# MarwanNour/SEAL-FYP-Logistic-Regression

Measured on AMD Instinct MI355X. Metric: CKKS ciphertext rotate+plain-mult ops/sec at N=16384; HBM GB/s vs roofline, higher is better.
Workload: dtype u64; 1 GPU; C3: N=16384, coeff_modulus bits [60, 40, 40, 40, 40, 60], level L=5 (k=6); per step and per GPU 4608 independent rotate_vector(step=1, direct Galois key)+multiply_plain, uniform random residues drawn on the device, inputs resident in HBM; batch_per_gpu=4608, parallelism=1 x independent ciphertext batches (no data-path collective), algorithmic_bytes_per_op=11141120

## Files before the change

seal_fyp_logistic_regression_amd/csrc/hefx_capi.cpp:

```cpp
#include "../../include/hefx.h"

#include <chrono>
#include <cmath>
#include <cstdio>
#include <cstring>
#include <map>
#include <mutex>
#include <tuple>
#include <string>
#include <unordered_map>
#include <unordered_set>
#include <algorithm>
#include <functional>
#include <vector>

#include <dlfcn.h>
#include <link.h>

#include "hefx_internal.h"

using namespace hefx;
typedef unsigned __int128 u128;

static thread_local std::string g_err;
// ... 981 lines not shown
        if (e == hipSuccess) rc = ntt_common(c, false, (uint64_t *)(rows + per * i0), cnt, c->k, 0, (void *)s);
    }
    if (e == hipSuccess && rc == HEFX_OK) e = hipStreamSynchronize(s);
    if (e != hipSuccess || rc != HEFX_OK) {
        (void)hipFree(rows);
        return rc != HEFX_OK ? rc : hipfail(e, "flip-mask tables");
    }
    std::lock_guard<std::mutex> lk(c->mu);
    c->flipw_slabs.push_back(rows);
    c->flipw_bytes += per * miss.size() * sizeof(u64);
    for (size_t i = 0; i < miss.size(); ++i) c->flipw.emplace(miss[i], rows + per * i);
    resolve();
    return HEFX_OK;
}

static size_t ks_words_per_item(const hefx_context *c, int L)
{
    return (size_t)c->n * ((size_t)L + 2 * (size_t)(L + 1) + 2);
}
static size_t ks_x_words(const hefx_context *c, int L, int items) { return (size_t)c->n * items * L * (L + 1); }

static int ks_small_shape(int n, int L)
{
    static const int quarter_force = getenv("HEFX_QUARTER") ? atoi(getenv("HEFX_QUARTER")) : -1;
    static const int qmask_force = getenv("HEFX_QMASK") ? atoi(getenv("HEFX_QMASK")) : -1;
    static const int pair_force = getenv("HEFX_PAIR") ? atoi(getenv("HEFX_PAIR")) : -1;
    if (qmask_force >= 0) return qmask_force & (KS_Q_ALL | KS_Q_PAIR);
    if (pair_force > 0 || (pair_force < 0 && quarter_force < 0 && n * L * L * 4 <= 256)) return KS_Q_PAIR;
    if (quarter_force >= 0) return quarter_force ? KS_Q_ALL : 0;
    return (n * L * 4 <= 256 ? KS_Q_INTT : 0) | (n * L * L * 4 <= 256 ? KS_Q_NTT : 0) | (n * 2 * 4 <= 256 ? KS_Q_MDI : 0) |
           (n * 2 * L * 4 <= 320 ? KS_Q_FIN : 0);
// ... 6 lines not shown
{
    CTXCHK(c);
    static const bool ksdbg = getenv("HEFX_DEBUG") && atoi(getenv("HEFX_DEBUG")) >= 2;
    const auto ks_t0 = std::chrono::steady_clock::now();
    auto ks_us = [&] { return std::chrono::duration<double, std::micro>(std::chrono::steady_clock::now() - ks_t0).count(); };
    double t_valid = 0, t_tables = 0;
    if (int rc = check_ks_level(c, L)) return rc;
    if (n < 1 || !ct_in || !ct_out) return fail(HEFX_ERR_INVALID, "bad key-switch batch arguments");
    if (!relin && (!elts || !keys)) return fail(HEFX_ERR_INVALID, "missing Galois elements / keys");
    if (relin && !single_key) return fail(HEFX_ERR_INVALID, "missing relinearization key");
    if ((acc_in != nullptr) != (acc_out != nullptr) || (acc_out && (relin || pts || hoist)))
        return fail(HEFX_ERR_INVALID, "accumulate: rotations only, input and output sums together, no fused plaintext");
    const size_t per = ks_words_per_item(c, L);
    int chunk = c->chunk;
    if (chunk <= 0) {
        chunk = (int)(((size_t)1 << 30) / (per * sizeof(u64)));
        const int cap = c->logn <= 13 ? 2 * KS_AUTO_CHUNK : KS_AUTO_CHUNK;
        chunk = chunk > cap ? cap : (chunk < 16 ? 16 : chunk & ~7);
    }
    const int nchunks = (n + chunk - 1) / chunk;
    const bool two = nchunks > 1 && c->use_streams && !c->profiling;
    if (hoist) {
        if (relin) return fail(HEFX_ERR_INVALID, "hoisting applies to rotations only");
        for (int i = 0; i < n; ++i)
            if (ct_in[i] != ct_in[0] || ct_out[i] == ct_in[0])
                return fail(HEFX_ERR_INVALID, "hoisted batch: one shared source, never overwritten");
    }
    std::vector<const uint32_t *> perms(relin ? 0 : (size_t)n);
    bool any_alias = false;
    for (int i = 0; i < n; ++i) {
        if (!ct_in[i] || !ct_out[i]) return fail(HEFX_ERR_INVALID, "null ciphertext pointer in batch");
// ... 112 lines not shown
    }
    int ci = 0;
    ++c->stat_ks_calls;
    for (int base = 0; base < n && herr == hipSuccess; base += chunk, ++ci) {
        const int cnt = (n - base < chunk) ? n - base : chunk;
        const unsigned slot = c->ring_next++ % KS_RING;
        if (c->ring_busy[slot]) {
            KS_TRY(hipEventSynchronize(c->ring_ev[slot]));
            c->ring_busy[slot] = false;
        }
        KsItem *hb = c->h_items + (size_t)slot * KS_MAX_CHUNK, *db = c->d_items + (size_t)slot * KS_MAX_CHUNK;
        KsScratch S{};
        S.d = c->scratch + scratch_off + (two ? (size_t)(ci % ns) * half_words : 0);
        S.acc = S.d + (size_t)cnt * L * N;
        S.u = S.acc + (size_t)cnt * 2 * (L + 1) * N;
        S.x = S.u + (size_t)cnt * 2 * N;
        S.alias = S.x + ks_x_words(c, L, cnt);
        S.qmod = c->d_qmod;
        S.gate = c->d_gate + slot;
        S.gate_hits = c->d_gate + KS_RING;
        if (++c->gate_seq == 0) c->gate_seq = 1;
        S.gate_tag = c->gate_seq;
        S.gate_mode = 0;
        bool chunk_alias = false;
        int nsrc = 0;
        std::unordered_map<const void *, uint32_t> src_of;
        if (share && cnt > ks_small_max() && one_source && cnt + 1 <= KS_MAX_CHUNK) {
            src_of.emplace((const void *)ct_in[0], 0u);
            nsrc = 1;
        } else if (share && cnt > ks_small_max()) {
            for (int i = 0; i < cnt && src_of.size() * share_ratio <= (size_t)cnt; ++i)
// ... 189 lines not shown
        KsScratch S;
        KsItem *dbA, *dbB;
        hipStream_t s;
    };
    Lane lane[MAX_LANES];
    size_t off = 0;
    for (int l = 0; l < nl; ++l) {
        Lane &ln = lane[l];
        ln.lo = (int)((long long)n * l / nl);
        ln.cnt = (int)((long long)n * (l + 1) / nl) - ln.lo;
        ln.quarter = ks_small_shape(ln.cnt, L);
        ln.S = KsScratch{};
        ln.S.d = c->scratch + off;
        ln.S.acc = ln.S.d + (size_t)ln.cnt * L * N;
        ln.S.u = ln.S.acc + (size_t)ln.cnt * 2 * (L + 1) * N;
        ln.S.x = ln.S.u + (size_t)ln.cnt * 2 * N;
        ln.S.alias = ln.S.x + ks_x_words(c, L, ln.cnt);
        off += per * (size_t)ln.cnt + ks_x_words(c, L, ln.cnt);
        ln.dbA = c->chain_items + (size_t)l * 128;
        ln.dbB = ln.dbA + 64;
        ln.s = l == 0 ? user : c->streams[l - 1];
    }
    hipError_t herr = hipSuccess;
    if (nl > 1) {
        herr = hipEventRecord(c->ev_fork, user);
        for (int l = 1; l < nl && herr == hipSuccess; ++l) herr = hipStreamWaitEvent(lane[l].s, c->ev_fork, 0);
    }
    auto lane_level = [&](const Lane &ln, const uint64_t *const *in, uint64_t *const *out, KsItem *db) {
        return chain_level(c, L, ln.cnt, in + ln.lo, out + ln.lo, acc_out + ln.lo, acc_out + ln.lo, elts + ln.lo, keys + ln.lo,
                           perms.data() + ln.lo, ln.S, db, ln.quarter, ln.s);
    };
// ... 576 lines not shown
            for (int q = 1; q < LANES; ++q)
                if (load[q] < load[ln]) ln = q;
            root_lane[(size_t)r] = (uint8_t)ln;
            load[ln] += weight[(size_t)r];
        }
        std::vector<int> cnt((size_t)max_depth * LANES, 0);
        int widest = 0;
        for (size_t i = 0; i < nodes.size(); ++i) {
            lane_of[i] = root_lane[(size_t)root_of[i]];
            widest = std::max(widest, ++cnt[(size_t)nodes[i].depth * LANES + lane_of[i]]);
        }
        bool all_loaded = true;
        for (int q = 0; q < LANES; ++q) all_loaded = all_loaded && load[q] > 0;
        int chunk = c->chunk;
        if (chunk <= 0) {
            chunk = (int)(((size_t)1 << 30) / (ks_words_per_item(c, L) * sizeof(u64)));
            const int cap = c->logn <= 13 ? 2 * KS_AUTO_CHUNK : KS_AUTO_CHUNK;
            chunk = chunk > cap ? cap : (chunk < 16 ? 16 : chunk & ~7);
        }
        if (all_loaded && widest <= chunk) {
            lane1_off = ks_words_per_item(c, L) * (size_t)widest + ks_x_words(c, L, widest);
            if (int rc = ensure_scratch(c, (size_t)LANES * lane1_off)) return rc;
            nlanes = LANES;
            std::vector<uint32_t> all_elts(nodes.size());
            for (size_t i = 0; i < nodes.size(); ++i) all_elts[i] = nodes[i].elt;
            std::sort(all_elts.begin(), all_elts.end());
            all_elts.erase(std::unique(all_elts.begin(), all_elts.end()), all_elts.end());
            std::vector<const u64 *> unused;
            if (int rc = ensure_flipw(c, all_elts.data(), (int)all_elts.size(), (hipStream_t)stream, unused)) return rc;
            for (uint32_t e : all_elts) {
                const uint32_t *perm = nullptr;
// ... 354 lines not shown
        if (int rc = ks_run(c, L, 1, false, &src, &first[t], &key, nullptr, nullptr, &dst, stream)) return rc;
        src = dst;
    }
    if (int rc = hefx_add(c, L, 2, 1, ct, src, ct_new, stream)) return rc;
    if (int rc = hefx_multiply_plain(c, L, 2, 1, ct_new, diag_pts_keylevel[0], cbuf, stream)) return rc;
    if (nrot == 0) {
        HIPCHK(hipMemcpyAsync(out, cbuf, ctw * sizeof(u64), hipMemcpyDeviceToDevice, (hipStream_t)stream));
        return HEFX_OK;
    }
    const size_t per = ks_words_per_item(c, L) + ks_x_words(c, L, 1);
    if (int rc = ensure_scratch(c, per)) return rc;
    KsScratch S{};
    S.d = c->scratch;
    S.acc = S.d + (size_t)L * N;
    S.u = S.acc + (size_t)2 * (L + 1) * N;
    S.x = S.u + (size_t)2 * N;
    S.alias = nullptr;
    hipStream_t s = (hipStream_t)stream;
    HIPCHK(hipMemcpyAsync(d_items, items.data(), sizeof(KsItem) * items.size(), hipMemcpyHostToDevice, s));
    HIPCHK(hipStreamSynchronize(s));
    HIPCHK(launch_lt2_decompose(c->T, L, d_items, d_items + 1, nrot, S, (const u64 *)ct_new, partial_s, partial_c0,
                                (u64 *)cbuf, s));
    HIPCHK(launch_lt2_moddown(c->T, L, d_items + nterms, S, s));
    return HEFX_OK;
}

extern "C" int hefx_linear_transform_plain_hoisted2(hefx_context *c, int L, const uint64_t *ct, int d,
                                                    const uint64_t *const *diag_pts_keylevel, int nkeys,
                                                    const uint32_t *key_elts, const uint64_t *const *keys,
                                                    uint64_t *out, void *stream)
{
// ... 243 lines not shown
```

seal_fyp_logistic_regression_amd/csrc/hefx_keyswitch.hip:

```cpp
#include <cstdio>
#include <cstdlib>
#include "hefx_internal.h"
#include "hefx_ntt.cuh"
#include "hefx_ntt8.cuh"

template <int LOGN>
struct KsWaves {
    static constexpr int INV = LOGN <= 14 ? 2 : 4;
    static constexpr int FWD = LOGN <= 13 ? 2 : 4;
    static constexpr int NB_INV = (INV <= 2 && LOGN <= 13) ? 1 : 2, NB_FWD = (FWD <= 2 && LOGN < 13) ? 1 : 2;
    static constexpr bool PARITY_CUT = true;
};

namespace hefx {

typedef u64 u64x2_t __attribute__((ext_vector_type(2)));
__device__ __forceinline__ ulonglong2 nt_load16(const u64 *p)
{
    const u64x2_t v = __builtin_nontemporal_load(reinterpret_cast<const u64x2_t *>(p));
    return make_ulonglong2(v.x, v.y);
}
__device__ __forceinline__ void nt_store16(u64 *p, u64 a, u64 b)
{
    u64x2_t v;
    v.x = a, v.y = b;
    __builtin_nontemporal_store(v, reinterpret_cast<u64x2_t *>(p));
// ... 715 lines not shown
    const size_t w = (size_t)blockIdx.x * blockDim.x + threadIdx.x;
    u64 xl = 0, xh = 0, yl = 0, yh = 0;
    const int l0 = ch * LT2_CHUNK, l1 = l0 + LT2_CHUNK < nrot ? l0 + LT2_CHUNK : nrot;
    const u64 *__restrict__ row = c0 + (size_t)j * n;
    for (int l = l0; l < l1; ++l) {
        const KsItem it = items[l];
        const uint2 pi = gld_u32x2(it.perm + 2 * w);
        const ulonglong2 dg = gld16(it.pt + (size_t)j * n + 2 * w);
        mac128(xl, xh, gld8(row + pi.x), dg.x);
        mac128(yl, yh, gld8(row + pi.y), dg.y);
    }
    reinterpret_cast<ulonglong2 *>(partial + ((size_t)ch * L + j) * n)[w] =
        make_ulonglong2(barrett128(xl, xh, mc), barrett128(yl, yh, mc));
}

template <int LOGN>
__global__ __launch_bounds__(SplitCfg<LOGN>::T, KsWaves<LOGN>::INV) void ks_moddown_intt_kernel(DevTables T, int L, int rows,
                                                                               KsScratch S)
{
    using SC = SplitCfg<LOGN>;
    using C = typename SC::C;
    extern __shared__ __align__(16) u64 lds[];
    HEFX_STAMP_KERNEL(3);
    HEFX_STAMP_AT(0);
    int p, h;
    split_decode(blockIdx.x, p, h);
    if (p >= rows || (S.gate_mode == 2 && ks_gated_out(S))) return;
    const int t = threadIdx.x;
    const int sp = T.k - 1;
    const ModConst mc = T.mods[sp];
    const ulonglong2 *__restrict__ src =
        reinterpret_cast<const ulonglong2 *>(S.acc + ((size_t)p * (L + 1) + L) * SC::N);
    u64 v[16];
    split_inv<LOGN, KsWaves<LOGN>::NB_INV>(v, src, lds, ntt_tables(T, sp), mc, T.modsf[sp], t, h);
    const u64 half = mc.q >> 1;
    u64 *__restrict__ ud = S.u + (size_t)p * SC::N + (size_t)h * SC::H;
#pragma unroll
    for (int r = 0; r < 16; ++r) ud[C::idx_nat(t, r)] = csub(v[r] + half, mc.q);
    HEFX_STAMP_AT(15);
}

struct PinvU {
    ulonglong2 v;
};
struct PinvF {
    double2 v;
};
template <bool L16>
__device__ __forceinline__ PinvU md_pinv(ArithU64T<L16>, const DevTables &T, int sp, int j)
{
    return PinvU{T.invmod[(size_t)sp * T.k + j]};
}
__device__ __forceinline__ PinvF md_pinv(ArithF64, const DevTables &T, int sp, int j)
// ... 1 lines not shown
    return PinvF{T.invmodf[(size_t)sp * T.k + j]};
}
template <bool L16>
__device__ __forceinline__ u64 md_epilogue(ArithU64T<L16>, u64 f, u64 acc, u64 sadd, u64 pt, bool has_pt,
                                           const typename ArithU64T<L16>::Ctx &cx, const PinvU &pinv, const ModConst &mc)
{
    return ArithU64T<L16>::moddown(f, acc, sadd, pt, has_pt, cx, pinv.v, mc);
}
__device__ __forceinline__ u64 md_epilogue(ArithF64, double f, u64 acc, u64 sadd, u64 pt, bool has_pt,
                                           const ArithF64::Ctx &cx, const PinvF &pinv, const ModConst &)
{
    return ArithF64::moddown(f, acc, sadd, pt, has_pt, cx, pinv.v);
}

template <int LOGN, class A>
__device__ __forceinline__ void moddown_finish_body(const DevTables &T, const KsItem &it, int L, int relin,
                                                    const KsScratch &S, u64 *lds,
                                                    const typename A::TW *__restrict__ tw, const typename A::Ctx &cx,
                                                    const ModConst &mc, int b, int c, int j, int t, int h)
{
    using SC = SplitCfg<LOGN>;
    using C = typename SC::C;
    const int sp = T.k - 1;
    const u64 q = mc.q;
    const u64 half_j = T.halfmod[(size_t)sp * T.k + j];
    const auto pinv = md_pinv(A{}, T, sp, j);
    const u64 *__restrict__ ud = S.u + ((size_t)b * 2 + c) * SC::N;
    const InMode mode = {true, true, true, half_j, true, T.mods[sp].q < 2 * mc.q};
    const int tl = HEFX_EO_LANE(SC, t);
    auto ld = [&](int r, u64 &x, u64 &y) {
        const uint32_t e = eo_nat<SC>(tl, r);
        x = ud[e];
        y = ud[e + SC::H / 2];
    };
    const size_t off = (size_t)h * SC::H;
    const u64 *__restrict__ acc = S.acc + (((size_t)b * 2 + c) * (L + 1) + j) * SC::N + off;
    const u64 *__restrict__ addrow = it.c_in + ((size_t)(relin ? c : 0) * L + j) * SC::N;
    const bool has_add = relin || c == 0;
    const uint32_t elt = relin ? 1u : item_elt(it);
    const u64 *__restrict__ pt = it.pt ? it.pt + (size_t)j * SC::N + off : nullptr;
    u64 *__restrict__ dst = it.c_out + ((size_t)c * L + j) * SC::N + off;
    typename A::V f[16];
    u64 keep[16];
    {
        constexpr int GS = 4, NG = 16 / GS;
        constexpr bool PIPE = KsWaves<LOGN>::FWD <= 2;
        constexpr int NBUF = PIPE ? 2 : 1;
        static_assert(GS % 2 == 0, "record layout");
        split_fwd_raw<LOGN, A, decltype(ld), KsWaves<LOGN>::NB_FWD, NoHook, true>(f, ld, mode, mc, lds, tw, cx, t, h, NoHook(), tl);
        auto epilogue = [&](auto has_add_c, auto has_pt_c) {
            constexpr bool HA = decltype(has_add_c)::value, HP = decltype(has_pt_c)::value;
            u64 a[NBUF][GS], sadd[NBUF][GS], pp[NBUF][GS];
            auto fetch = [&](int g, int bufi) {
#pragma unroll
                for (int r = 0; r < GS; r += 2) {
                    const int idx = C::idx_io(t, GS * g + r);
                    const ulonglong2 av = gld16(acc + idx);
                    ulonglong2 sv = make_ulonglong2(0, 0), pv = make_ulonglong2(0, 0);
                    if constexpr (HA) sv = gather_pair(addrow, (uint32_t)((off + idx) >> 1), elt, LOGN);
                    if constexpr (HP) pv = gld16(pt + idx);
                    a[bufi][r] = av.x, a[bufi][r + 1] = av.y;
                    sadd[bufi][r] = sv.x, sadd[bufi][r + 1] = sv.y;
                    pp[bufi][r] = pv.x, pp[bufi][r + 1] = pv.y;
                }
// ... 27 lines not shown
        }
        if (it.acc_out && !pt) {
            const size_t arow = ((size_t)c * L + j) * SC::N + off;
            const u64 *__restrict__ ain = it.acc_in + arow;
            u64 *__restrict__ aout = it.acc_out + arow;
            ulonglong2 av[8];
#pragma unroll
            for (int r = 0; r < 16; r += 2) av[r / 2] = gld16(ain + C::idx_io(t, r));
#pragma unroll
            for (int r = 0; r < 16; r += 2)
                gst16(aout + C::idx_io(t, r), make_ulonglong2(addmod(av[r / 2].x, keep[r], q), addmod(av[r / 2].y, keep[r + 1], q)));
        }
    }
}

template <int LOGN>
__global__ __launch_bounds__(SplitCfg<LOGN>::T, KsWaves<LOGN>::FWD) void ks_moddown_finish_kernel(DevTables T,
                                                                                 const KsItem *__restrict__ items, int L,
                                                                                 int relin, int rows, KsScratch S)
{
    extern __shared__ __align__(16) u64 lds[];
    HEFX_STAMP_KERNEL(4);
    HEFX_STAMP_AT(0);
    int g, j, h;
    group_decode(blockIdx.x, L, g, j, h);
    if (g >= rows || ks_gated_out(S)) return;
    const int t = threadIdx.x;
    const int b = g >> 1, c = g & 1;
    const ModConst mc = T.mods[j];
    const ModConstF mf = T.modsf[j];
    const NttTables nt = ntt_tables(T, j);
    const KsItem it = items[b];
    if (mf.q != 0.0)
        moddown_finish_body<LOGN, ArithF64>(T, it, L, relin, S, lds, nt.twf, ArithF64::make(mf), mc, b, c, j, t, h);
    else
        moddown_finish_body<LOGN, ArithU64>(T, it, L, relin, S, lds, nt.tw, ArithU64::make(mc), mc, b, c, j, t, h);
    HEFX_STAMP_AT(15);
}

template <int LOGN>
struct QuarterCfg {
    using C = Ntt8Cfg<LOGN - 2>;
    static constexpr int N = 1 << LOGN;
    static constexpr int Q = N / 4;
    static constexpr int T = C::T;
    static constexpr size_t LDS_BYTES = sizeof(u64) * C::LDS_WORDS;
};
__host__ __device__ static inline int quarter_grid(int rows) { return ((rows + 7) / 8) * 32; }
__device__ static __forceinline__ void quarter_decode(int bid, int &p, int &part)
{
    part = 3 - ((bid >> 3) & 3);
// ... 548 lines not shown
{
    using SC = SplitCfg<LOGN>;
    constexpr bool CUT = KsWaves<LOGN>::PARITY_CUT;
    const int stream_x = may_stream && (size_t)n * L * (L + 1) * SC::N * 8 > ((size_t)256 << 20) ? 1 : 0;
    mark(2);
    hipLaunchKernelGGL((ks_ntt_digits_kernel<LOGN, CUT>), dim3(group_grid(n * L, L)), dim3(SC::T), SC::LDS_BYTES, s, T, L,
                       n * L, stream_x | order_flags, scr);
    mark(3);
    const dim3 grid(SC::N / 2 / 256, L + 1, (n + 1) / 2);
    if (stream_x)
        hipLaunchKernelGGL((ks_mac_kernel<true, CUT>), grid, dim3(256), 0, s, T, batch, L, rl, n, scr);
    else
        hipLaunchKernelGGL((ks_mac_kernel<false, CUT>), grid, dim3(256), 0, s, T, batch, L, rl, n, scr);
}

template <int LOGN>
static hipError_t launch_keyswitch_chunk_t(const DevTables &T, int L, int n, const KsItem *batch, bool relin,
                                           const KsScratch &scr, bool alias, const KsSmallItems *small, int quarter,
                                           hipStream_t s, KsProf *prof, int nsrc)
{
    using SC = SplitCfg<LOGN>;
    const size_t lds = SC::LDS_BYTES;
    static PerDeviceOnce attr_once;
    if (attr_once.first()) {
        set_lds(ks_intt_digits_kernel<LOGN>, lds);
        set_lds(ks_intt_digits_small_kernel<LOGN>, lds);
        set_lds(ks_ntt_digits_kernel<LOGN>, lds);
        set_lds(ks_ntt_digits_kernel<LOGN, KsWaves<LOGN>::PARITY_CUT>, lds);
        set_lds(ks_moddown_intt_kernel<LOGN>, lds);
        set_lds(ks_moddown_finish_kernel<LOGN>, lds);
        if (getenv("HEFX_DEBUG")) {
            int nb = -1;
            (void)hipOccupancyMaxActiveBlocksPerMultiprocessor(&nb, ks_ntt_digits_kernel<LOGN, KsWaves<LOGN>::PARITY_CUT>,
                                                               SC::T, lds);
            fprintf(stderr, "[hefx] ks_ntt_digits_kernel<%d, %d>: %d threads, %zu B LDS -> %d workgroups/CU\n", LOGN,
                    (int)KsWaves<LOGN>::PARITY_CUT, SC::T, lds, nb);
        }
    }
    const int rl = relin ? 1 : 0;
    auto mark = [&](int stage) {
        if (prof && prof->used < prof->cap) {
            (void)hipEventRecord(prof->ev[prof->used], s);
            prof->stage[prof->used++] = stage;
        }
    };
    if (nsrc > 0) {
        KsScratch hs = scr, fb = scr;
        hs.gate_mode = 1;
        fb.gate_mode = 2;
        mark(1);
        hipLaunchKernelGGL((ks_intt_digits_kernel<LOGN>), dim3(split_grid(nsrc * L)), dim3(SC::T), lds, s, T, batch + n, L,
                           0, 1, nsrc * L, hs);
        mark(2);
        hipLaunchKernelGGL((ks_ntt_digits_kernel<LOGN>), dim3(group_grid(nsrc * L, L)), dim3(SC::T), lds, s, T, L, nsrc * L, 0,
                           hs);
        mark(3);
        hipLaunchKernelGGL(ks_mac_exact_kernel, dim3(SC::N / 2 / 256, L + 1, n), dim3(256), 0, s, T, batch, L, hs);
        mark(4);
        hipLaunchKernelGGL((ks_moddown_intt_kernel<LOGN>), dim3(split_grid(n * 2)), dim3(SC::T), lds, s, T, L, n * 2, hs);
        mark(5);
        hipLaunchKernelGGL((ks_moddown_finish_kernel<LOGN>), dim3(group_grid(n * 2, L)), dim3(SC::T), lds, s, T, batch, L,
                           0, n * 2, hs);
        mark(7);
        hipLaunchKernelGGL((ks_intt_digits_kernel<LOGN>), dim3(split_grid(n * L)), dim3(SC::T), lds, s, T, batch, L, 0, 0,
                           n * L, fb);
        hipLaunchKernelGGL((ks_ntt_digits_kernel<LOGN>), dim3(group_grid(n * L, L)), dim3(SC::T), lds, s, T, L, n * L, 0, fb);
        hipLaunchKernelGGL(ks_mac_kernel<false>, dim3(SC::N / 2 / 256, L + 1, (n + 1) / 2), dim3(256), 0, s, T, batch, L, 0, n,
                           fb);
        hipLaunchKernelGGL((ks_moddown_intt_kernel<LOGN>), dim3(split_grid(n * 2)), dim3(SC::T), lds, s, T, L, n * 2, fb);
        hipLaunchKernelGGL((ks_moddown_finish_kernel<LOGN>), dim3(group_grid(n * 2, L)), dim3(SC::T), lds, s, T, batch, L,
                           0, n * 2, fb);
        mark(-1);
        return hipGetLastError();
    }
    if (small && (quarter & KS_Q_PAIR)) {
        static PerDeviceOnce attrp;
        const size_t ldsq = QuarterCfg<LOGN>::LDS_BYTES;
        if (attrp.first()) {
            set_lds(ks_pair_digits_kernel<LOGN>, ldsq);
            set_lds(ks_pair_moddown_kernel<LOGN>, ldsq);
        }
        constexpr int TQ = QuarterCfg<LOGN>::T;
        mark(1);
        hipLaunchKernelGGL((ks_pair_digits_kernel<LOGN>), fan_grid(n * L, 4 * L), dim3(TQ), ldsq, s, T, *small,
                           const_cast<KsItem *>(batch), n, L, rl, n * L, scr);
        mark(3);
// ... 23 lines not shown
        if (quarter & KS_Q_INTT)
            hipLaunchKernelGGL((ks_intt_digits_q_kernel<LOGN>), dim3(quarter_grid(n * L)), dim3(TQ), ldsq, s, T, *small,
                               const_cast<KsItem *>(batch), n, L, rl, n * L, scr);
        else
            hipLaunchKernelGGL((ks_intt_digits_small_kernel<LOGN>), dim3(split_grid(n * L)), dim3(SC::T), lds, s, T, *small,
                               const_cast<KsItem *>(batch), n, L, rl, n * L, scr);
        if (quarter & KS_Q_NTT) {
            mark(2);
            hipLaunchKernelGGL((ks_ntt_digits_q_kernel<LOGN>), fan_grid(n * L, 4 * L), dim3(TQ), ldsq, s, T, L,
                               n * L, scr);
            mark(3);
            hipLaunchKernelGGL(ks_mac_kernel<false>, dim3(SC::N / 2 / 256, L + 1, (n + 1) / 2), dim3(256), 0, s, T, batch, L,
                               rl, n, scr);
        } else
            launch_digits_and_mac<LOGN>(T, L, n, batch, rl, heavy_order, false, scr, s, mark);
        mark(4);
        if (quarter & KS_Q_MDI)
            hipLaunchKernelGGL((ks_moddown_intt_q_kernel<LOGN>), dim3(quarter_grid(n * 2)), dim3(TQ), ldsq, s, T, L, n * 2,
                               scr);
        else
            hipLaunchKernelGGL((ks_moddown_intt_kernel<LOGN>), dim3(split_grid(n * 2)), dim3(SC::T), lds, s, T, L, n * 2,
                               scr);
        mark(5);
        if (quarter & KS_Q_FIN)
            hipLaunchKernelGGL((ks_moddown_finish_q_kernel<LOGN>), fan_grid(n * 2, 4 * L), dim3(TQ), ldsq, s, T,
                               batch, L, rl, n * 2, scr);
        else
            hipLaunchKernelGGL((ks_moddown_finish_kernel<LOGN>), dim3(group_grid(n * 2, L)), dim3(SC::T), lds, s, T,
                               batch, L, rl, n * 2, scr);
        mark(-1);
        return hipGetLastError();
    }
    if (alias) {
        mark(0);
        hipLaunchKernelGGL(ks_alias_copy_kernel, dim3(SC::N / 2 / 256, 2 * L, n), dim3(256), 0, s, T, batch, L);
    }
    mark(1);
    if (small)
        hipLaunchKernelGGL((ks_intt_digits_small_kernel<LOGN>), dim3(split_grid(n * L)), dim3(SC::T), lds, s, T, *small,
                           const_cast<KsItem *>(batch), n, L, rl, n * L, scr);
    else
        hipLaunchKernelGGL((ks_intt_digits_kernel<LOGN>), dim3(split_grid(n * L)), dim3(SC::T), lds, s, T, batch, L, rl, 0,
                           n * L, scr);
    launch_digits_and_mac<LOGN>(T, L, n, batch, rl, heavy_order, true, scr, s, mark);
    mark(4);
    hipLaunchKernelGGL((ks_moddown_intt_kernel<LOGN>), dim3(split_grid(n * 2)), dim3(SC::T), lds, s, T, L, n * 2, scr);
    mark(5);
    hipLaunchKernelGGL((ks_moddown_finish_kernel<LOGN>), dim3(group_grid(n * 2, L)), dim3(SC::T), lds, s, T, batch, L,
                       rl, n * 2, scr);
    mark(-1);
    return hipGetLastError();
}

__global__ __launch_bounds__(256) void lt2_reduce_kernel(DevTables T, int L, int period, int rows, int chunks,
                                                         const u64 *__restrict__ partial, const u64 *addin, u64 *out)
{
    const size_t n = (size_t)1 << T.logn;
    const int r = blockIdx.y;
    const int jj = r % period;
    const u64 q = T.mods[jj < L ? jj : T.k - 1].q;
    const size_t w = (size_t)blockIdx.x * blockDim.x + threadIdx.x;
    ulonglong2 acc = addin ? reinterpret_cast<const ulonglong2 *>(addin + (size_t)r * n)[w] : make_ulonglong2(0, 0);
    for (int ch = 0; ch < chunks; ++ch) {
        const ulonglong2 v = reinterpret_cast<const ulonglong2 *>(partial + ((size_t)ch * rows + r) * n)[w];
// ... 4 lines not shown
        acc = make_ulonglong2(ArithF64::raw(ArithF64::from_u64(acc.x)), ArithF64::raw(ArithF64::from_u64(acc.y)));
    reinterpret_cast<ulonglong2 *>(out + (size_t)r * n)[w] = acc;
}

template <int LOGN>
static hipError_t launch_lt2_decompose_t(const DevTables &T, int L, const KsItem *src_item, const KsItem *rot_items,
                                         int nrot, const KsScratch &scr, const u64 *ct_new, u64 *partial_s,
                                         u64 *partial_c0, u64 *cbuf, hipStream_t s)
{
    using SC = SplitCfg<LOGN>;
    const size_t lds = SC::LDS_BYTES;
    static PerDeviceOnce attr_once;
    if (attr_once.first()) {
        set_lds(ks_intt_digits_kernel<LOGN>, lds);
        set_lds(ks_ntt_digits_kernel<LOGN>, lds);
        set_lds(ks_moddown_intt_kernel<LOGN>, lds);
        set_lds(ks_moddown_finish_kernel<LOGN>, lds);
    }
    const int chunks = (nrot + LT2_CHUNK - 1) / LT2_CHUNK;
    hipLaunchKernelGGL((ks_intt_digits_kernel<LOGN>), dim3(split_grid(L)), dim3(SC::T), lds, s, T, src_item, L, 0, 1, L,
                       scr);
    hipLaunchKernelGGL((ks_ntt_digits_kernel<LOGN>), dim3(group_grid(L, L)), dim3(SC::T), lds, s, T, L, L, 0, scr);
    hipLaunchKernelGGL(lt2_mac_kernel, dim3(SC::N / 2 / 256, L + 1, chunks), dim3(256), 0, s, T, rot_items, L, nrot, scr,
                       ct_new + (size_t)L * SC::N, partial_s);
    hipLaunchKernelGGL(lt2_c0_kernel, dim3(SC::N / 2 / 256, L, chunks), dim3(256), 0, s, T, rot_items, L, nrot, ct_new,
                       partial_c0);
    hipLaunchKernelGGL(lt2_reduce_kernel, dim3(SC::N / 2 / 256, 2 * (L + 1)), dim3(256), 0, s, T, L, L + 1, 2 * (L + 1),
                       chunks, partial_s, (const u64 *)nullptr, scr.acc);
    hipLaunchKernelGGL(lt2_reduce_kernel, dim3(SC::N / 2 / 256, L), dim3(256), 0, s, T, L, L, L, chunks, partial_c0,
                       (const u64 *)cbuf, cbuf);
    return hipGetLastError();
}
template <int LOGN>
static hipError_t launch_lt2_moddown_t(const DevTables &T, int L, const KsItem *item, const KsScratch &scr, hipStream_t s)
{
    using SC = SplitCfg<LOGN>;
    const size_t lds = SC::LDS_BYTES;
    hipLaunchKernelGGL((ks_moddown_intt_kernel<LOGN>), dim3(split_grid(2)), dim3(SC::T), lds, s, T, L, 2, scr);
    hipLaunchKernelGGL((ks_moddown_finish_kernel<LOGN>), dim3(group_grid(2, L)), dim3(SC::T), lds, s, T, item, L, 1, 2,
                       scr);
    return hipGetLastError();
}

#ifdef HEFX_ONLY_LOGN
#define HEFX_DISPATCH_SPLIT(logn, CALL) \
    if ((logn) == HEFX_ONLY_LOGN) return CALL(HEFX_ONLY_LOGN); \
    return hipErrorInvalidValue;
#else
#define HEFX_DISPATCH_SPLIT(logn, CALL)       \
    switch (logn) {                           \
        case 11: return CALL(11);             \
        case 12: return CALL(12);             \
        case 13: return CALL(13);             \
        case 14: return CALL(14);             \
        case 15: return CALL(15);             \
// ... 219 lines not shown
```

seal_fyp_logistic_regression_amd/csrc/hefx_ntt.cuh:

```cuda
#pragma once
#include <type_traits>

#include "hefx_modarith.cuh"

#ifdef HEFX_STAMP
namespace hefx {
static __device__ u64 hefx_stamp_buf[8 * 1024 * 16];
__device__ __forceinline__ int &hefx_stamp_kid()
{
    __shared__ int kid;
    return kid;
}
}
#define HEFX_STAMP_KERNEL(k) do { if (threadIdx.x == 0) hefx_stamp_kid() = (k); } while (0)
#define HEFX_STAMP_AT(id)                                                                                            \
    do {                                                                                                             \
        if (HEFX_STAMP > 1) asm volatile("s_waitcnt vmcnt(0) lgkmcnt(0)" ::: "memory");                              \
        const unsigned hefx_wg_ = blockIdx.x + gridDim.x * (blockIdx.y + gridDim.y * blockIdx.z);                   \
        if (threadIdx.x == 0 && hefx_wg_ < 1024)                                                                     \
            hefx_stamp_buf[((size_t)hefx_stamp_kid() * 1024 + hefx_wg_) * 16 + (id)] = wall_clock64();               \
    } while (0)
#else
#define HEFX_STAMP_KERNEL(k) do { } while (0)
#define HEFX_STAMP_AT(id) do { } while (0)
// ... 79 lines not shown
        u64 t = shoup_lazy4(y, w.x, w.y, c.nq);
        x = a + t;
        y = a + c.four_q - t;
    }
    __device__ static __forceinline__ TW half_twiddle(const TW &w, const Ctx &c, int h)
    {
        TW r;
        r.x = h ? c.q - w.x : w.x;
        r.y = h ? ~w.y : w.y;
        return r;
    }
    __device__ static __forceinline__ V ct_half(V x, V y, const TW &wh, const Ctx &c)
    {
        return x + shoup_lazy4(y, wh.x, wh.y, c.nq);
    }
    __device__ static __forceinline__ void gs(V &x, V &y, const TW &w, const Ctx &c)
    {
        u64 s = csubn(x + y, c.n4q);
        u64 d = x + c.four_q - y;
        x = s;
        y = shoup_lazy4(d, w.x, w.y, c.nq);
    }
    __device__ static __forceinline__ void gs_last(V &x, V &y, const Ctx &c)
    {
        u64 s = x + y;
        u64 d = x + c.four_q - y;
        x = shoup_lazy(s, c.ninv, c.ninv_s, c.nq);
        y = shoup_lazy(d, c.ilw, c.ilw_s, c.nq);
    }
    __device__ static __forceinline__ V gs_half_sum(V a0, V a1, const Ctx &) { return a0 + a1; }
// ... 91 lines not shown
        return s + l;
    }
    __device__ static __forceinline__ double red(double x, const Ctx &c)
    {
        return __builtin_fma(-__builtin_rint(x * c.qinv), c.q, x);
    }
    __device__ static __forceinline__ void ct(V &x, V &y, const TW &w, const Ctx &c, int )
    {
        const double t = mm(y, w, c);
        const double a = x;
        x = a + t;
        y = a - t;
    }
    __device__ static __forceinline__ TW half_twiddle(const TW &w, const Ctx &, int h) { return h ? -w : w; }
    __device__ static __forceinline__ V ct_half(V x, V y, const TW &wh, const Ctx &c) { return x + mm(y, wh, c); }
    __device__ static __forceinline__ void gs(V &x, V &y, const TW &w, const Ctx &c)
    {
        const double s = x + y, d = x - y;
        x = s;
        y = mm(d, w, c);
    }
    __device__ static __forceinline__ void gs_last(V &x, V &y, const Ctx &c)
    {
        const double s = x + y, d = x - y;
        x = mm(s, c.ninv, c);
        y = mm(d, c.ilw, c);
    }
    __device__ static __forceinline__ V gs_half_sum(V a0, V a1, const Ctx &) { return a0 + a1; }
    __device__ static __forceinline__ V gs_half_diff(V a0, V a1, const TW &w, const Ctx &c)
    {
// ... 360 lines not shown
        }
    }
    ntt_fwd_core<LOGN - 1, A, HOOK>(f, reinterpret_cast<typename A::V *>(lds), tw, cx, t, 2 + h, tail_hook, t0);
    using C = NttCfg<LOGN - 1>;
    if constexpr (C::R == 0) {
        typename A::V *lf = reinterpret_cast<typename A::V *>(lds);
        const int pw = 17 * t, pr = 2 * t + (t >> 3);
#pragma unroll
        for (int r = 0; r < 16; ++r) lf[pw + r] = f[r];
        __syncthreads();
#pragma unroll
        for (int r = 0; r < 16; ++r) f[r] = lf[pr + (2 * C::T + C::T / 8) * (r >> 1) + (r & 1)];
    }
}

template <int LOGN, class A, class LD, int NB = 2, bool MACOP = false>
__device__ __forceinline__ void split_fwd_a(u64 (&v)[16], const LD &ld, const InMode &mode, const ModConst &mc,
                                            u64 *lds, const typename A::TW *__restrict__ tw,
                                            const typename A::Ctx &cx, int t, int h, int t0 = -1, int mac_slack = 0)
{
    typename A::V f[16];
    split_fwd_raw<LOGN, A, LD, NB>(f, ld, mode, mc, lds, tw, cx, t, h, NoHook(), t0);
    if (MACOP && !A::IS_F64 && mac_slack == 1) {
#pragma unroll
        for (int r = 0; r < 16; ++r) v[r] = A::template mac_operand_lazy<1>(f[r], cx);
    } else if (MACOP && !A::IS_F64 && mac_slack >= 2) {
#pragma unroll
        for (int r = 0; r < 16; ++r) v[r] = A::template mac_operand_lazy<2>(f[r], cx);
    } else {
#pragma unroll
// ... 146 lines not shown
```

Before: 252,200 rotate+multiply_plain ops/s.

## Prestage first forward NTT butterfly of moddown into the INTT kernel

The moddown INTT kernel now reduces its output for every target prime j, applies the first forward-NTT butterfly stage there, and writes L per-prime half-transformed rows into an enlarged u buffer. The finish kernel then loads these prestaged rows (non-temporal for large batches) and runs only the remaining NTT stages, instead of each of the L finish blocks reloading the shared u row and redoing the first stage. Scratch layout grows the u region from 2N to 2LN words per item, while the chunk-size rule keeps the old formula. This trades extra HBM writes and scratch for removing the split first stage and its LDS exchange in the finish kernel.

```diff
diff --git a/seal_fyp_logistic_regression_amd/csrc/hefx_capi.cpp b/seal_fyp_logistic_regression_amd/csrc/hefx_capi.cpp
--- a/seal_fyp_logistic_regression_amd/csrc/hefx_capi.cpp
+++ b/seal_fyp_logistic_regression_amd/csrc/hefx_capi.cpp
@@ -1019,7 +1019,12 @@
     return HEFX_OK;
 }
 
+static size_t ks_u_words(const hefx_context *c, int L, int items) { return (size_t)c->n * items * 2 * (size_t)L; }
 static size_t ks_words_per_item(const hefx_context *c, int L)
+{
+    return (size_t)c->n * ((size_t)L + 2 * (size_t)(L + 1)) + ks_u_words(c, L, 1);
+}
+static size_t ks_rule_words_per_item(const hefx_context *c, int L)
 {
     return (size_t)c->n * ((size_t)L + 2 * (size_t)(L + 1) + 2);
 }
@@ -1056,7 +1061,7 @@
     const size_t per = ks_words_per_item(c, L);
     int chunk = c->chunk;
     if (chunk <= 0) {
-        chunk = (int)(((size_t)1 << 30) / (per * sizeof(u64)));
+        chunk = (int)(((size_t)1 << 30) / (ks_rule_words_per_item(c, L) * sizeof(u64)));
         const int cap = c->logn <= 13 ? 2 * KS_AUTO_CHUNK : KS_AUTO_CHUNK;
         chunk = chunk > cap ? cap : (chunk < 16 ? 16 : chunk & ~7);
     }
@@ -1199,7 +1204,7 @@
         S.d = c->scratch + scratch_off + (two ? (size_t)(ci % ns) * half_words : 0);
         S.acc = S.d + (size_t)cnt * L * N;
         S.u = S.acc + (size_t)cnt * 2 * (L + 1) * N;
-        S.x = S.u + (size_t)cnt * 2 * N;
+        S.x = S.u + ks_u_words(c, L, cnt);
         S.alias = S.x + ks_x_words(c, L, cnt);
         S.qmod = c->d_qmod;
         S.gate = c->d_gate + slot;
@@ -1419,7 +1424,7 @@
         ln.S.d = c->scratch + off;
         ln.S.acc = ln.S.d + (size_t)ln.cnt * L * N;
         ln.S.u = ln.S.acc + (size_t)ln.cnt * 2 * (L + 1) * N;
-        ln.S.x = ln.S.u + (size_t)ln.cnt * 2 * N;
+        ln.S.x = ln.S.u + ks_u_words(c, L, ln.cnt);
         ln.S.alias = ln.S.x + ks_x_words(c, L, ln.cnt);
         off += per * (size_t)ln.cnt + ks_x_words(c, L, ln.cnt);
         ln.dbA = c->chain_items + (size_t)l * 128;
@@ -2026,7 +2031,7 @@
         for (int q = 0; q < LANES; ++q) all_loaded = all_loaded && load[q] > 0;
         int chunk = c->chunk;
         if (chunk <= 0) {
-            chunk = (int)(((size_t)1 << 30) / (ks_words_per_item(c, L) * sizeof(u64)));
+            chunk = (int)(((size_t)1 << 30) / (ks_rule_words_per_item(c, L) * sizeof(u64)));
             const int cap = c->logn <= 13 ? 2 * KS_AUTO_CHUNK : KS_AUTO_CHUNK;
             chunk = chunk > cap ? cap : (chunk < 16 ? 16 : chunk & ~7);
         }
@@ -2411,7 +2416,7 @@
     S.d = c->scratch;
     S.acc = S.d + (size_t)L * N;
     S.u = S.acc + (size_t)2 * (L + 1) * N;
-    S.x = S.u + (size_t)2 * N;
+    S.x = S.u + ks_u_words(c, L, 1);
     S.alias = nullptr;
     hipStream_t s = (hipStream_t)stream;
     HIPCHK(hipMemcpyAsync(d_items, items.data(), sizeof(KsItem) * items.size(), hipMemcpyHostToDevice, s));
diff --git a/seal_fyp_logistic_regression_amd/csrc/hefx_keyswitch.hip b/seal_fyp_logistic_regression_amd/csrc/hefx_keyswitch.hip
--- a/seal_fyp_logistic_regression_amd/csrc/hefx_keyswitch.hip
+++ b/seal_fyp_logistic_regression_amd/csrc/hefx_keyswitch.hip
@@ -10,6 +10,7 @@
     static constexpr int FWD = LOGN <= 13 ? 2 : 4;
     static constexpr int NB_INV = (INV <= 2 && LOGN <= 13) ? 1 : 2, NB_FWD = (FWD <= 2 && LOGN < 13) ? 1 : 2;
     static constexpr bool PARITY_CUT = true;
+    static constexpr bool MD_PRESTAGE = true;
 };
 
 namespace hefx {
@@ -755,9 +756,32 @@
         make_ulonglong2(barrett128(xl, xh, mc), barrett128(yl, yh, mc));
 }
 
-template <int LOGN>
+template <int LOGN, class A, int RED>
+__device__ __forceinline__ void md_prestage_store(const u64 (&v)[16], const InMode &mode, const ModConst &mcj,
+                                                  const typename A::Ctx &cx, const typename A::TW &w, u64 *__restrict__ dx,
+                                                  u64 *__restrict__ dy, bool stream)
+{
+    constexpr int T = SplitCfg<LOGN>::T;
+#pragma unroll
+    for (int m = 0; m < 4; ++m) {
+        typename A::V X[2], Y[2];
+#pragma unroll
+        for (int e = 0; e < 2; ++e)
+            A::ct_half_both(A::template input<RED>(v[2 * m + e], mode, cx, mcj),
+                            A::template input<RED>(v[2 * m + e + 8], mode, cx, mcj), w, cx, X[e], Y[e]);
+        if (stream) {
+            nt_store16(dx + 2 * T * m, A::raw(X[0]), A::raw(X[1]));
+            nt_store16(dy + 2 * T * m, A::raw(Y[0]), A::raw(Y[1]));
+        } else {
+            gst16(dx + 2 * T * m, make_ulonglong2(A::raw(X[0]), A::raw(X[1])));
+            gst16(dy + 2 * T * m, make_ulonglong2(A::raw(Y[0]), A::raw(Y[1])));
+        }
+    }
+}
+
+template <int LOGN, bool PRE = false>
 __global__ __launch_bounds__(SplitCfg<LOGN>::T, KsWaves<LOGN>::INV) void ks_moddown_intt_kernel(DevTables T, int L, int rows,
-                                                                               KsScratch S)
+                                                                               KsScratch S, int stream_u)
 {
     using SC = SplitCfg<LOGN>;
     using C = typename SC::C;
@@ -775,9 +799,38 @@
     u64 v[16];
     split_inv<LOGN, KsWaves<LOGN>::NB_INV>(v, src, lds, ntt_tables(T, sp), mc, T.modsf[sp], t, h);
     const u64 half = mc.q >> 1;
-    u64 *__restrict__ ud = S.u + (size_t)p * SC::N + (size_t)h * SC::H;
-#pragma unroll
-    for (int r = 0; r < 16; ++r) ud[C::idx_nat(t, r)] = csub(v[r] + half, mc.q);
+    if constexpr (!PRE) {
+        u64 *__restrict__ ud = S.u + (size_t)p * SC::N + (size_t)h * SC::H;
+#pragma unroll
+        for (int r = 0; r < 16; ++r) ud[C::idx_nat(t, r)] = csub(v[r] + half, mc.q);
+    } else {
+#pragma unroll
+        for (int r = 0; r < 16; ++r) v[r] = csub(v[r] + half, mc.q);
+#pragma unroll 1
+        for (int j = 0; j < L; ++j) {
+#pragma unroll
+            for (int r = 0; r < 16; ++r) asm volatile("" : "+v"(v[r]));
+            const ModConst mcj = T.mods[j];
+            const ModConstF mfj = T.modsf[j];
+            const InMode mode = {true, true, true, T.halfmod[(size_t)sp * T.k + j], true, mc.q < 2 * mcj.q};
+            const NttTables nt = ntt_tables(T, j);
+            u64 *__restrict__ dx = S.u + ((size_t)p * L + j) * SC::N + (size_t)h * (SC::H / 2) + 2 * t;
+            u64 *__restrict__ dy = dx + SC::H;
+            if (mfj.q != 0.0) {
+                const ArithF64::Ctx cx = ArithF64::make(mfj);
+                if (mode.below_2_61 && ArithF64::fast_wide(cx))
+                    md_prestage_store<LOGN, ArithF64, 2>(v, mode, mcj, cx, nt.twf[1], dx, dy, stream_u != 0);
+                else
+                    md_prestage_store<LOGN, ArithF64, 1>(v, mode, mcj, cx, nt.twf[1], dx, dy, stream_u != 0);
+            } else {
+                const ArithU64::Ctx cx = ArithU64::make(mcj);
+                if (LOGN >= 14 && mode.lt2q)
+                    md_prestage_store<LOGN, ArithU64, 3>(v, mode, mcj, cx, nt.tw[1], dx, dy, stream_u != 0);
+                else
+                    md_prestage_store<LOGN, ArithU64, 1>(v, mode, mcj, cx, nt.tw[1], dx, dy, stream_u != 0);
+            }
+        }
+    }
     HEFX_STAMP_AT(15);
 }
 
@@ -809,10 +862,30 @@
 }
 
 template <int LOGN, class A>
+__device__ __forceinline__ void md_prestage_load(typename A::V (&f)[16], const u64 *__restrict__ half_row, int t, bool stream)
+{
+    constexpr int T = SplitCfg<LOGN>::T;
+    const u64 *__restrict__ src = half_row + (size_t)(t / (T / 2)) * (SplitCfg<LOGN>::H / 2) + 2 * (t & (T / 2 - 1));
+    ulonglong2 rec[8];
+#pragma unroll
+    for (int a = 0; a < 2; ++a)
+#pragma unroll
+        for (int m = 0; m < 4; ++m)
+            rec[4 * a + m] = stream ? nt_load16(src + 2 * T * m + T * a) : gld16(src + 2 * T * m + T * a);
+#pragma unroll
+    for (int a = 0; a < 2; ++a)
+#pragma unroll
+        for (int m = 0; m < 4; ++m) {
+            f[4 * m + a] = A::unraw(rec[4 * a + m].x);
+            f[4 * m + 2 + a] = A::unraw(rec[4 * a + m].y);
+        }
+}
+
+template <int LOGN, class A, bool PRE>
 __device__ __forceinline__ void moddown_finish_body(const DevTables &T, const KsItem &it, int L, int relin,
                                                     const KsScratch &S, u64 *lds,
                                                     const typename A::TW *__restrict__ tw, const typename A::Ctx &cx,
-                                                    const ModConst &mc, int b, int c, int j, int t, int h)
+                                                    const ModConst &mc, int b, int c, int j, int t, int h, bool stream_u)
 {
     using SC = SplitCfg<LOGN>;
     using C = typename SC::C;
@@ -842,7 +915,11 @@
         constexpr bool PIPE = KsWaves<LOGN>::FWD <= 2;
         constexpr int NBUF = PIPE ? 2 : 1;
         static_assert(GS % 2 == 0, "record layout");
-        split_fwd_raw<LOGN, A, decltype(ld), KsWaves<LOGN>::NB_FWD, NoHook, true>(f, ld, mode, mc, lds, tw, cx, t, h, NoHook(), tl);
+        if constexpr (PRE) {
+            md_prestage_load<LOGN, A>(f, S.u + ((((size_t)b * 2 + c) * L + j) * 2 + h) * SC::H, t, stream_u);
+            split_fwd_staged<LOGN, A>(f, lds, tw, cx, t, h, eo_lane<SC>(t));
+        } else
+            split_fwd_raw<LOGN, A, decltype(ld), KsWaves<LOGN>::NB_FWD, NoHook, true>(f, ld, mode, mc, lds, tw, cx, t, h, NoHook(), tl);
         auto epilogue = [&](auto has_add_c, auto has_pt_c) {
             constexpr bool HA = decltype(has_add_c)::value, HP = decltype(has_pt_c)::value;
             u64 a[NBUF][GS], sadd[NBUF][GS], pp[NBUF][GS];
@@ -900,10 +977,11 @@
     }
 }
 
-template <int LOGN>
+template <int LOGN, bool PRE = false>
 __global__ __launch_bounds__(SplitCfg<LOGN>::T, KsWaves<LOGN>::FWD) void ks_moddown_finish_kernel(DevTables T,
                                                                                  const KsItem *__restrict__ items, int L,
-                                                                                 int relin, int rows, KsScratch S)
+                                                                                 int relin, int rows, KsScratch S,
+                                                                                 int stream_u)
 {
     extern __shared__ __align__(16) u64 lds[];
     HEFX_STAMP_KERNEL(4);
@@ -918,9 +996,11 @@
     const NttTables nt = ntt_tables(T, j);
     const KsItem it = items[b];
     if (mf.q != 0.0)
-        moddown_finish_body<LOGN, ArithF64>(T, it, L, relin, S, lds, nt.twf, ArithF64::make(mf), mc, b, c, j, t, h);
+        moddown_finish_body<LOGN, ArithF64, PRE>(T, it, L, relin, S, lds, nt.twf, ArithF64::make(mf), mc, b, c, j, t, h,
+                                                 stream_u != 0);
     else
-        moddown_finish_body<LOGN, ArithU64>(T, it, L, relin, S, lds, nt.tw, ArithU64::make(mc), mc, b, c, j, t, h);
+        moddown_finish_body<LOGN, ArithU64, PRE>(T, it, L, relin, S, lds, nt.tw, ArithU64::make(mc), mc, b, c, j, t, h,
+                                                 stream_u != 0);
     HEFX_STAMP_AT(15);
 }
 
@@ -1499,6 +1579,32 @@
         hipLaunchKernelGGL((ks_mac_kernel<false, CUT>), grid, dim3(256), 0, s, T, batch, L, rl, n, scr);
 }
 
+struct NoMark {
+    void operator()(int) const {}
+};
+template <int LOGN, class MARK = NoMark>
+static void launch_moddown(const DevTables &T, int L, int n, const KsItem *batch, int rl, bool may_stream,
+                           const KsScratch &scr, hipStream_t s, const MARK &mark = MARK())
+{
+    using SC = SplitCfg<LOGN>;
+    constexpr bool PRE = KsWaves<LOGN>::MD_PRESTAGE;
+    const int stream_u = PRE && may_stream && (size_t)n * L * (L + 1) * SC::N * 8 > ((size_t)256 << 20) ? 1 : 0;
+    mark(4);
+    hipLaunchKernelGGL((ks_moddown_intt_kernel<LOGN, PRE>), dim3(split_grid(n * 2)), dim3(SC::T), SC::LDS_BYTES, s, T, L,
+                       n * 2, scr, stream_u);
+    mark(5);
+    hipLaunchKernelGGL((ks_moddown_finish_kernel<LOGN, PRE>), dim3(group_grid(n * 2, L)), dim3(SC::T), SC::LDS_BYTES, s, T,
+                       batch, L, rl, n * 2, scr, stream_u);
+}
+template <int LOGN>
+static void set_lds_moddown(size_t lds)
+{
+    set_lds(ks_moddown_intt_kernel<LOGN, false>, lds);
+    set_lds(ks_moddown_finish_kernel<LOGN, false>, lds);
+    set_lds(ks_moddown_intt_kernel<LOGN, KsWaves<LOGN>::MD_PRESTAGE>, lds);
+    set_lds(ks_moddown_finish_kernel<LOGN, KsWaves<LOGN>::MD_PRESTAGE>, lds);
+}
+
 template <int LOGN>
 static hipError_t launch_keyswitch_chunk_t(const DevTables &T, int L, int n, const KsItem *batch, bool relin,
                                            const KsScratch &scr, bool alias, const KsSmallItems *small, int quarter,
@@ -1512,8 +1618,7 @@
         set_lds(ks_intt_digits_small_kernel<LOGN>, lds);
         set_lds(ks_ntt_digits_kernel<LOGN>, lds);
         set_lds(ks_ntt_digits_kernel<LOGN, KsWaves<LOGN>::PARITY_CUT>, lds);
-        set_lds(ks_moddown_intt_kernel<LOGN>, lds);
-        set_lds(ks_moddown_finish_kernel<LOGN>, lds);
+        set_lds_moddown<LOGN>(lds);
         if (getenv("HEFX_DEBUG")) {
             int nb = -1;
             (void)hipOccupancyMaxActiveBlocksPerMultiprocessor(&nb, ks_ntt_digits_kernel<LOGN, KsWaves<LOGN>::PARITY_CUT>,
@@ -1541,20 +1646,14 @@
                            hs);
         mark(3);
         hipLaunchKernelGGL(ks_mac_exact_kernel, dim3(SC::N / 2 / 256, L + 1, n), dim3(256), 0, s, T, batch, L, hs);
-        mark(4);
-        hipLaunchKernelGGL((ks_moddown_intt_kernel<LOGN>), dim3(split_grid(n * 2)), dim3(SC::T), lds, s, T, L, n * 2, hs);
-        mark(5);
-        hipLaunchKernelGGL((ks_moddown_finish_kernel<LOGN>), dim3(group_grid(n * 2, L)), dim3(SC::T), lds, s, T, batch, L,
-                           0, n * 2, hs);
+        launch_moddown<LOGN>(T, L, n, batch, 0, true, hs, s, mark);
         mark(7);
         hipLaunchKernelGGL((ks_intt_digits_kernel<LOGN>), dim3(split_grid(n * L)), dim3(SC::T), lds, s, T, batch, L, 0, 0,
                            n * L, fb);
         hipLaunchKernelGGL((ks_ntt_digits_kernel<LOGN>), dim3(group_grid(n * L, L)), dim3(SC::T), lds, s, T, L, n * L, 0, fb);
         hipLaunchKernelGGL(ks_mac_kernel<false>, dim3(SC::N / 2 / 256, L + 1, (n + 1) / 2), dim3(256), 0, s, T, batch, L, 0, n,
                            fb);
-        hipLaunchKernelGGL((ks_moddown_intt_kernel<LOGN>), dim3(split_grid(n * 2)), dim3(SC::T), lds, s, T, L, n * 2, fb);
-        hipLaunchKernelGGL((ks_moddown_finish_kernel<LOGN>), dim3(group_grid(n * 2, L)), dim3(SC::T), lds, s, T, batch, L,
-                           0, n * 2, fb);
+        launch_moddown<LOGN>(T, L, n, batch, 0, true, fb, s);
         mark(-1);
         return hipGetLastError();
     }
@@ -1608,20 +1707,25 @@
                                rl, n, scr);
         } else
             launch_digits_and_mac<LOGN>(T, L, n, batch, rl, heavy_order, false, scr, s, mark);
+        if (!(quarter & (KS_Q_MDI | KS_Q_FIN))) {
+            launch_moddown<LOGN>(T, L, n, batch, rl, false, scr, s, mark);
+            mark(-1);
+            return hipGetLastError();
+        }
         mark(4);
         if (quarter & KS_Q_MDI)
             hipLaunchKernelGGL((ks_moddown_intt_q_kernel<LOGN>), dim3(quarter_grid(n * 2)), dim3(TQ), ldsq, s, T, L, n * 2,
                                scr);
         else
-            hipLaunchKernelGGL((ks_moddown_intt_kernel<LOGN>), dim3(split_grid(n * 2)), dim3(SC::T), lds, s, T, L, n * 2,
-                               scr);
+            hipLaunchKernelGGL((ks_moddown_intt_kernel<LOGN, false>), dim3(split_grid(n * 2)), dim3(SC::T), lds, s, T, L,
+                               n * 2, scr, 0);
         mark(5);
         if (quarter & KS_Q_FIN)
             hipLaunchKernelGGL((ks_moddown_finish_q_kernel<LOGN>), fan_grid(n * 2, 4 * L), dim3(TQ), ldsq, s, T,
                                batch, L, rl, n * 2, scr);
         else
-            hipLaunchKernelGGL((ks_moddown_finish_kernel<LOGN>), dim3(group_grid(n * 2, L)), dim3(SC::T), lds, s, T,
-                               batch, L, rl, n * 2, scr);
+            hipLaunchKernelGGL((ks_moddown_finish_kernel<LOGN, false>), dim3(group_grid(n * 2, L)), dim3(SC::T), lds, s, T,
+                               batch, L, rl, n * 2, scr, 0);
         mark(-1);
         return hipGetLastError();
     }
@@ -1637,11 +1741,7 @@
         hipLaunchKernelGGL((ks_intt_digits_kernel<LOGN>), dim3(split_grid(n * L)), dim3(SC::T), lds, s, T, batch, L, rl, 0,
                            n * L, scr);
     launch_digits_and_mac<LOGN>(T, L, n, batch, rl, heavy_order, true, scr, s, mark);
-    mark(4);
-    hipLaunchKernelGGL((ks_moddown_intt_kernel<LOGN>), dim3(split_grid(n * 2)), dim3(SC::T), lds, s, T, L, n * 2, scr);
-    mark(5);
-    hipLaunchKernelGGL((ks_moddown_finish_kernel<LOGN>), dim3(group_grid(n * 2, L)), dim3(SC::T), lds, s, T, batch, L,
-                       rl, n * 2, scr);
+    launch_moddown<LOGN>(T, L, n, batch, rl, true, scr, s, mark);
     mark(-1);
     return hipGetLastError();
 }
@@ -1676,8 +1776,7 @@
     if (attr_once.first()) {
         set_lds(ks_intt_digits_kernel<LOGN>, lds);
         set_lds(ks_ntt_digits_kernel<LOGN>, lds);
-        set_lds(ks_moddown_intt_kernel<LOGN>, lds);
-        set_lds(ks_moddown_finish_kernel<LOGN>, lds);
+        set_lds_moddown<LOGN>(lds);
     }
     const int chunks = (nrot + LT2_CHUNK - 1) / LT2_CHUNK;
     hipLaunchKernelGGL((ks_intt_digits_kernel<LOGN>), dim3(split_grid(L)), dim3(SC::T), lds, s, T, src_item, L, 0, 1, L,
@@ -1696,11 +1795,7 @@
 template <int LOGN>
 static hipError_t launch_lt2_moddown_t(const DevTables &T, int L, const KsItem *item, const KsScratch &scr, hipStream_t s)
 {
-    using SC = SplitCfg<LOGN>;
-    const size_t lds = SC::LDS_BYTES;
-    hipLaunchKernelGGL((ks_moddown_intt_kernel<LOGN>), dim3(split_grid(2)), dim3(SC::T), lds, s, T, L, 2, scr);
-    hipLaunchKernelGGL((ks_moddown_finish_kernel<LOGN>), dim3(group_grid(2, L)), dim3(SC::T), lds, s, T, item, L, 1, 2,
-                       scr);
+    launch_moddown<LOGN>(T, L, 1, item, 1, false, scr, s);
     return hipGetLastError();
 }
 
diff --git a/seal_fyp_logistic_regression_amd/csrc/hefx_ntt.cuh b/seal_fyp_logistic_regression_amd/csrc/hefx_ntt.cuh
--- a/seal_fyp_logistic_regression_amd/csrc/hefx_ntt.cuh
+++ b/seal_fyp_logistic_regression_amd/csrc/hefx_ntt.cuh
@@ -117,6 +117,11 @@
     {
         return x + shoup_lazy4(y, wh.x, wh.y, c.nq);
     }
+    __device__ static __forceinline__ void ct_half_both(V x, V y, const TW &w, const Ctx &c, V &X, V &Y)
+    {
+        X = ct_half(x, y, half_twiddle(w, c, 0), c);
+        Y = ct_half(x, y, half_twiddle(w, c, 1), c);
+    }
     __device__ static __forceinline__ void gs(V &x, V &y, const TW &w, const Ctx &c)
     {
         u64 s = csubn(x + y, c.n4q);
@@ -238,6 +243,12 @@
     }
     __device__ static __forceinline__ TW half_twiddle(const TW &w, const Ctx &, int h) { return h ? -w : w; }
     __device__ static __forceinline__ V ct_half(V x, V y, const TW &wh, const Ctx &c) { return x + mm(y, wh, c); }
+    __device__ static __forceinline__ void ct_half_both(V x, V y, const TW &w, const Ctx &c, V &X, V &Y)
+    {
+        const double m = mm(y, w, c);
+        X = x + m;
+        Y = x - m;
+    }
     __device__ static __forceinline__ void gs(V &x, V &y, const TW &w, const Ctx &c)
     {
         const double s = x + y, d = x - y;
@@ -628,6 +639,23 @@
     }
 }
 
+template <int LOGN, class A>
+__device__ __forceinline__ void split_fwd_staged(typename A::V (&f)[16], u64 *lds, const typename A::TW *__restrict__ tw,
+                                                 const typename A::Ctx &cx, int t, int h, int t0)
+{
+    ntt_fwd_core<LOGN - 1, A>(f, reinterpret_cast<typename A::V *>(lds), tw, cx, t, 2 + h, NoHook(), t0);
+    using C = NttCfg<LOGN - 1>;
+    if constexpr (C::R == 0) {
+        typename A::V *lf = reinterpret_cast<typename A::V *>(lds);
+        const int pw = 17 * t, pr = 2 * t + (t >> 3);
+#pragma unroll
+        for (int r = 0; r < 16; ++r) lf[pw + r] = f[r];
+        __syncthreads();
+#pragma unroll
+        for (int r = 0; r < 16; ++r) f[r] = lf[pr + (2 * C::T + C::T / 8) * (r >> 1) + (r & 1)];
+    }
+}
+
 template <int LOGN, class A, class LD, int NB = 2, bool MACOP = false>
 __device__ __forceinline__ void split_fwd_a(u64 (&v)[16], const LD &ld, const InMode &mode, const ModConst &mc,
                                             u64 *lds, const typename A::TW *__restrict__ tw,
```

New measurement: 239,700 rotate+multiply_plain ops/s. 0.95x the previous value.
